# binli123/dsmil-wsi

Hardware: AMD Instinct MI355X
Metric: bags/sec aggregated (10kx512) (higher is better)
Workload: dtype f32; 1 GPU; DSMIL aggregator forward (FCLayer+BClassifier), c16 weights C=1, 64 bags x 10000 x 512 fp32 per GPU per pass, HBM-resident; bags_per_pass_per_gpu=64, rows=10000, feats=512, classes=1, tile_rows=128, parallelism=bag-sharded x1, streams=3, distinct_batches=3, logits_form=1, device_cus=256, persistent_grid=256

## Files before the change

dsmil-wsi_amd/csrc/agg_fwd.hip:

```cpp

#include <hip/hip_runtime.h>
#include <stdint.h>
#include <math.h>
#include <stdio.h>
#include <stdlib.h>
#include <string.h>
#include <atomic>
#include "dsmil_hip.h"
#include "prof.h"

#include "agg_common.h"
#include "agg_split.h"
#include "agg_hs.h"
#include "agg_f2.h"
#include "agg_f3.h"
#include "agg_res.h"
#include "lds_attr.h"

namespace {

template <int VEC, bool GIVEN, typename T = float>
__device__ __forceinline__ void logits_tile(
    const T* __restrict__ feats, const int64_t* __restrict__ offsets,
    const float* __restrict__ fc_w, const float* __restrict__ fc_b,
// ... 220 lines not shown
            a1 += b1;
            if (want_max) {
#pragma unroll
                for (int m = 1; m < 8; m <<= 1) xm = fmaxf(xm, __shfl_xor(xm, m, 64));
                if (j == 0 && rbase + rr < Nb) rowmax[off0 + r] = xm;
            }
            if (j == 0 && rbase + rr < Nb) {
                float* o = classes_out + (off0 + r) * (long long)C;
                o[c0] = a0;
                if (CP == 2 && c1 != c0) o[c1] = a1;
            }
            if (better(a0, r, bv0, bi0)) { bv0 = a0; bi0 = r; }
            if (CP == 2 && better(a1, r, bv1, bi1)) { bv1 = a1; bi1 = r; }
        }
#pragma unroll
        for (int m = 8; m < 64; m <<= 1) {
            const float ov0 = __shfl_xor(bv0, m, 64);
            const long long oi0 = __shfl_xor(bi0, m, 64);
            if (better(ov0, oi0, bv0, bi0)) { bv0 = ov0; bi0 = oi0; }
            if constexpr (CP == 2) {
                const float ov1 = __shfl_xor(bv1, m, 64);
                const long long oi1 = __shfl_xor(bi1, m, 64);
                if (better(ov1, oi1, bv1, bi1)) { bv1 = ov1; bi1 = oi1; }
            }
        }
        __syncthreads();
        if (lane == 0) { s_v[wave] = bv0; s_i[wave] = bi0; s_v[4 + wave] = bv1; s_i[4 + wave] = bi1; }
        __syncthreads();
        if (tid < 2 && (tid == 0 || c1 != c0)) {
            const int h = tid * 4;
            float bv = s_v[h];
            long long bi = s_i[h];
            for (int w = 1; w < 4; ++w)
                if (better(s_v[h + w], s_i[h + w], bv, bi)) { bv = s_v[h + w]; bi = s_i[h + w]; }
            const int c = tid ? c1 : c0;
            part_val[slot * C + c] = bv;
            part_idx[slot * C + c] = bi;
        }
    }
}

template <int CP>
__global__ __launch_bounds__(256, 6) void k_logits_pipe(
    const bf16_t* __restrict__ feats, const int64_t* __restrict__ offsets,
    const float* __restrict__ fc_w, const float* __restrict__ fc_b, float* __restrict__ classes_out,
    float* __restrict__ part_val, long long* __restrict__ part_idx, int bag0,
    int r0, const int* __restrict__ tile_pre, int n_bags) {
    constexpr int K = 512, SEG = 64;
    __shared__ __attribute__((aligned(16))) float s_w[CP * K];
    __shared__ float s_v[8];
    __shared__ int s_i[8];
    int bag = bag0 + (int)blockIdx.y, tile = (int)blockIdx.x;
    if (tile_pre) {
        if ((int)blockIdx.x >= tile_pre[n_bags]) return;
        const int b = tile_owner(tile_pre, n_bags, (int)blockIdx.x);
        bag = bag0 + b;
        tile = (int)blockIdx.x - tile_pre[b];
    }
    const long long off0 = offsets[bag];
    const long long Nbl = offsets[bag + 1] - off0;
    const long long row0l = (long long)tile * r0;
    if (row0l >= Nbl) return;
    const int Nb = (int)Nbl, row0 = (int)row0l;
    const int tid = threadIdx.x, lane = tid & 63, wave = tid >> 6;
    const int j = lane & 7, rr = lane >> 3;
    const int ngrp = r0 >> 5, rpw = r0 >> 2;
    const int wbase = row0 + wave * rpw;
    int ng = 0;
    if (wbase < Nb) { const int left = (Nb - wbase + 7) >> 3; ng = left < ngrp ? left : ngrp; }
    for (int i = tid; i < CP * K; i += 256) s_w[i] = fc_w[i];
    __syncthreads();
    const float b0 = fc_b[0], b1 = fc_b[CP - 1];
    float bv0 = -INFINITY, bv1 = -INFINITY;
    int bi0 = 0x7fffffff, bi1 = 0x7fffffff;
    if (ng > 0) {
        typedef StreamVec<bf16_t> SV;
        const bf16_t* fbase = feats + j * 8;
        auto row_of = [&](int g) { const int r = wbase + g * 8 + rr; return r < Nb ? r : Nb - 1; };
        auto ptr_of = [&](int r) { return fbase + (off0 + r) * (long long)K; };
        SV va[4], vb[4];
        float a0 = 0.f, a1 = 0.f;
        const unsigned wad = (unsigned)(size_t)(__attribute__((address_space(3))) float*)s_w + j * 32;
        auto piece = [&](const SV& v, auto off_tag) {
            constexpr int OFF = decltype(off_tag)::value;
            f32x4 wa, wb, wc, wd;
            if constexpr (CP == 2) {
                asm volatile("ds_read_b128 %0, %6 offset:%7\n\tds_read_b128 %1, %6 offset:%8\n\t"
                             "ds_read_b128 %2, %6 offset:%9\n\tds_read_b128 %3, %6 offset:%10\n\ts_waitcnt lgkmcnt(0)"
                             : "=&v"(wa), "=&v"(wb), "=&v"(wc), "=&v"(wd), "+v"(a0), "+v"(a1)
                             : "v"(wad), "n"(OFF), "n"(OFF + 16), "n"(OFF + K * 4), "n"(OFF + K * 4 + 16) : "memory");
            } else {
                asm volatile("ds_read_b128 %0, %3 offset:%4\n\tds_read_b128 %1, %3 offset:%5\n\ts_waitcnt lgkmcnt(0)"
                             : "=&v"(wa), "=&v"(wb), "+v"(a0) : "v"(wad), "n"(OFF), "n"(OFF + 16) : "memory");
            }
#pragma unroll
            for (int e = 0; e < 4; ++e) a0 = fmaf(v.at(e), wa[e], a0);
#pragma unroll
            for (int e = 0; e < 4; ++e) a0 = fmaf(v.at(4 + e), wb[e], a0);
            if constexpr (CP == 2) {
#pragma unroll
                for (int e = 0; e < 4; ++e) a1 = fmaf(v.at(e), wc[e], a1);
#pragma unroll
                for (int e = 0; e < 4; ++e) a1 = fmaf(v.at(4 + e), wd[e], a1);
            }
        };
        auto consume_lo = [&](const SV (&v)[4]) {
            piece(v[0], std::integral_constant<int, 0 * 256>{}); piece(v[1], std::integral_constant<int, 1 * 256>{});
            piece(v[2], std::integral_constant<int, 2 * 256>{}); piece(v[3], std::integral_constant<int, 3 * 256>{});
        };
        auto consume_hi = [&](const SV (&v)[4]) {
            piece(v[0], std::integral_constant<int, 4 * 256>{}); piece(v[1], std::integral_constant<int, 5 * 256>{});
            piece(v[2], std::integral_constant<int, 6 * 256>{}); piece(v[3], std::integral_constant<int, 7 * 256>{});
        };
        auto finish_rows = [&](int g, int r) {
#pragma unroll
            for (int m = 1; m < 8; m <<= 1) {
                a0 += __shfl_xor(a0, m, 64);
                if constexpr (CP == 2) a1 += __shfl_xor(a1, m, 64);
            }
            a0 += b0;
            a1 += b1;
            if (j == 0 && wbase + g * 8 + rr < Nb) {
                float* o = classes_out + (off0 + r) * (long long)CP;
                o[0] = a0;
                if constexpr (CP == 2) o[1] = a1;
            }
            if (a0 > bv0 || (a0 == bv0 && r < bi0)) { bv0 = a0; bi0 = r; }
            if (CP == 2 && (a1 > bv1 || (a1 == bv1 && r < bi1))) { bv1 = a1; bi1 = r; }
            a0 = 0.f;
            a1 = 0.f;
        };
        int r = row_of(0);
        const bf16_t* x = ptr_of(r);
#pragma unroll
        for (int u = 0; u < 4; ++u) va[u].load(x + u * SEG);
#pragma unroll 1
        for (int g = 0; g + 1 < ng; ++g) {
            const int rn = row_of(g + 1);
            const bf16_t* xn = ptr_of(rn);
#pragma unroll
            for (int u = 0; u < 4; ++u) vb[u].load(x + (4 + u) * SEG);
            consume_lo(va);
#pragma unroll
            for (int u = 0; u < 4; ++u) va[u].load(xn + u * SEG);
            consume_hi(vb);
            finish_rows(g, r);
            r = rn;
            x = xn;
        }
#pragma unroll
        for (int u = 0; u < 4; ++u) vb[u].load(x + (4 + u) * SEG);
        consume_lo(va);
        consume_hi(vb);
        finish_rows(ng - 1, r);
    }
#pragma unroll
    for (int m = 8; m < 64; m <<= 1) {
        const float ov0 = __shfl_xor(bv0, m, 64);
        const int oi0 = __shfl_xor(bi0, m, 64);
        if (ov0 > bv0 || (ov0 == bv0 && oi0 < bi0)) { bv0 = ov0; bi0 = oi0; }
        if constexpr (CP == 2) {
            const float ov1 = __shfl_xor(bv1, m, 64);
            const int oi1 = __shfl_xor(bi1, m, 64);
            if (ov1 > bv1 || (ov1 == bv1 && oi1 < bi1)) { bv1 = ov1; bi1 = oi1; }
        }
    }
    if (lane == 0) { s_v[wave] = bv0; s_i[wave] = bi0; s_v[4 + wave] = bv1; s_i[4 + wave] = bi1; }
    __syncthreads();
    if (tid < CP) {
        const int h = tid * 4;
        float bv = s_v[h];
        int bi = s_i[h];
        for (int w = 1; w < 4; ++w)
            if (s_v[h + w] > bv || (s_v[h + w] == bv && s_i[h + w] < bi)) { bv = s_v[h + w]; bi = s_i[h + w]; }
        const long long slot = off0 / r0 + bag + tile;
        part_val[slot * CP + tid] = bv;
        part_idx[slot * CP + tid] = bi == 0x7fffffff ? 0x7fffffffffffffffLL : (long long)bi;
    }
}

template <int VEC, typename T = float, bool PRE = false>
__device__ __forceinline__ void qmax_block(
    const T* __restrict__ feats, const int64_t* __restrict__ offsets,
    const float* __restrict__ part_val, const long long* __restrict__ part_idx,
    const float* __restrict__ q0_w, const float* __restrict__ q0_b,
    const float* __restrict__ q2_w, const float* __restrict__ q2_b,
    float* __restrict__ qmax, int64_t* __restrict__ idx_out, int K, int C, int nonlinear,
    int bag, int c, float* s_v, long long* s_i, float* s_h, int mode = 0, float* __restrict__ best_val_out = nullptr,
    const int64_t* __restrict__ rowmap = nullptr, int r0 = R0) {
    const long long off0 = mode == 2 ? 0 : offsets[bag];
    const long long Nb = mode == 2 ? C : offsets[bag + 1] - off0;
    const int lane = threadIdx.x & 63, wave = threadIdx.x >> 6;
    const int nwv = (int)blockDim.x >> 6;
    const int upw = QD / nwv;
    const long long slot0 = off0 / r0 + bag;
    const long long ntile = mode == 2 ? 0 : (Nb + r0 - 1) / r0;
    f32x4 w1r[PRE ? 32 : 1];
    float w2r[PRE ? 32 : 1];
    bool pre = false;
    float bv = -INFINITY;
    long long bi = 0x7fffffffffffffffLL;
    long long t_next = threadIdx.x;
    if constexpr (PRE) {
        pre = K == 512 && nwv == 8 && nonlinear && VEC == 4;
        if (pre) {
            if (t_next < ntile) {
                bv = part_val[(slot0 + t_next) * C + c];
                bi = part_idx[(slot0 + t_next) * C + c];
                t_next += blockDim.x;
            }
            __builtin_amdgcn_sched_barrier(0);
#pragma unroll
            for (int jb = 0; jb < 2; ++jb)
#pragma unroll
                for (int kk = 0; kk < 2; ++kk)
#pragma unroll
                    for (int u = 0; u < 8; ++u)
                        w1r[(jb * 2 + kk) * 8 + u] = *reinterpret_cast<const f32x4*>(q0_w + (long long)(wave * 16 + jb * 8 + u) * 512 + kk * 256 + lane * 4);
#pragma unroll
            for (int jb = 0; jb < 2; ++jb)
#pragma unroll
                for (int u = 0; u < 8; ++u) {
                    const float* wr = q2_w + (long long)(wave * 16 + jb * 8 + u) * QD;
                    w2r[(jb * 8 + u) * 2] = wr[lane];
                    w2r[(jb * 8 + u) * 2 + 1] = wr[lane + 64];
                }
            __builtin_amdgcn_sched_barrier(0);
        }
    }
    for (long long t = t_next; t < ntile; t += blockDim.x) {
        const float v = part_val[(slot0 + t) * C + c];
        const long long i = part_idx[(slot0 + t) * C + c];
        if (better(v, i, bv, bi)) { bv = v; bi = i; }
    }
#pragma unroll
    for (int o = 32; o >= 1; o >>= 1) {
        const float ov = __shfl_xor(bv, o, 64);
        const long long oi = __shfl_xor(bi, o, 64);
        if (better(ov, oi, bv, bi)) { bv = ov; bi = oi; }
    }
    if (lane == 0) { s_v[wave] = bv; s_i[wave] = bi; }
    __syncthreads();
    bv = s_v[0]; bi = s_i[0];
    for (int w = 1; w < nwv; ++w)
        if (better(s_v[w], s_i[w], bv, bi)) { bv = s_v[w]; bi = s_i[w]; }
    long long best = mode == 2 ? c : bi;
    if (best < 0 || best >= Nb) best = 0;
    if (threadIdx.x == 0 && mode != 2) {
        idx_out[(long long)bag * C + c] = best;
        if (best_val_out) best_val_out[(long long)bag * C + c] = bv;
    }
    if (mode == 1) return;
    const T* x = feats + (mode == 2 ? best : phys_row(rowmap, off0 + best)) * (long long)K;
    if (PRE && pre) {
        const f32x4 xv0 = load4<VEC, T>(x, lane * 4, K), xv1 = load4<VEC, T>(x, 256 + lane * 4, K);
#pragma unroll
        for (int jb = 0; jb < 2; ++jb) {
            float acc[8] = {0.f, 0.f, 0.f, 0.f, 0.f, 0.f, 0.f, 0.f};
#pragma unroll
            for (int kk = 0; kk < 2; ++kk) {
                const f32x4 xv = kk ? xv1 : xv0;
#pragma unroll
                for (int u = 0; u < 8; ++u) {
                    const f32x4 wv = w1r[(jb * 2 + kk) * 8 + u];
#pragma unroll
                    for (int e = 0; e < 4; ++e) acc[u] = fmaf(xv[e], wv[e], acc[u]);
                }
            }
#pragma unroll
            for (int u = 0; u < 8; ++u) {
                const float a = fmaxf(wave_sum(acc[u]) + q0_b[wave * 16 + jb * 8 + u], 0.f);
                if (lane == 0) s_h[wave * 16 + jb * 8 + u] = a;
            }
        }
        __syncthreads();
        float* out = qmax + ((long long)bag * C + c) * QD;
        const float h0 = s_h[lane], h1 = s_h[lane + 64];
#pragma unroll
        for (int jb = 0; jb < 2; ++jb) {
            float acc[8];
#pragma unroll
            for (int u = 0; u < 8; ++u) acc[u] = fmaf(h0, w2r[(jb * 8 + u) * 2], h1 * w2r[(jb * 8 + u) * 2 + 1]);
#pragma unroll
            for (int u = 0; u < 8; ++u) {
                const float a = wave_sum(acc[u]) + q2_b[wave * 16 + jb * 8 + u];
                if (lane == 0) out[wave * 16 + jb * 8 + u] = tanhf(a);
            }
        }
        return;
    }
    for (int jb = 0; jb < upw; jb += 8) {
        float acc[8] = {0.f, 0.f, 0.f, 0.f, 0.f, 0.f, 0.f, 0.f};
        const float* wr = q0_w + (long long)(wave * upw + jb) * K;
        for (int k0 = 0; k0 < K; k0 += 256) {
            const int k = k0 + lane * 4;
            const f32x4 xv = load4<VEC, T>(x, k, K);
#pragma unroll
            for (int u = 0; u < 8; ++u) {
                const f32x4 wv = load4<VEC>(wr + (long long)u * K, k, K);
#pragma unroll
                for (int e = 0; e < 4; ++e) acc[u] = fmaf(xv[e], wv[e], acc[u]);
            }
        }
#pragma unroll
        for (int u = 0; u < 8; ++u) {
            float a = wave_sum(acc[u]) + q0_b[wave * upw + jb + u];
// ... 931 lines not shown
}

int dsmil_fc_forward_rows(const float* feats, int64_t total_rows, int32_t K, int32_t C, const float* fc_w,
                          const float* fc_b, float* classes, const int64_t* rowmap, void* stream) {
    if (!feats || !fc_w || !fc_b || !classes || total_rows <= 0 || K <= 0 || C <= 0) return DSMIL_E_INVALID;
    hipStream_t st = (hipStream_t)stream;
    long long blocks = (total_rows + 3) / 4;
    if (blocks > 4096) blocks = 4096;
    const bool v4 = (K % 4 == 0) && (((uintptr_t)feats | (uintptr_t)fc_w) % 16 == 0);
    if (v4) hipLaunchKernelGGL(k_fc<4>, dim3((unsigned)blocks), dim3(256), 0, st, feats, fc_w, fc_b, classes, (long long)total_rows, K, C, rowmap);
    else hipLaunchKernelGGL(k_fc<1>, dim3((unsigned)blocks), dim3(256), 0, st, feats, fc_w, fc_b, classes, (long long)total_rows, K, C, rowmap);
    return hipGetLastError() == hipSuccess ? DSMIL_OK : DSMIL_E_LAUNCH;
}

void dsmil_agg_forward_leftovers(void* ws, int32_t n_bags, int64_t total_rows, int32_t K, int32_t Kv, int32_t C,
                                 const void** packed_split, const float** qmax, const float** pred_part, int* pred_blocks) {
    const WsLayout L = ws_layout(n_bags, total_rows, total_rows, K, Kv, C, pick_nw(n_bags, total_rows) * 32);
    if (pred_part) *pred_part = (const float*)((char*)ws + L.pred_part);
    if (pred_blocks) *pred_blocks = (int)L.nchunk_max;
    if (packed_split) *packed_split = (pick_nw(n_bags, total_rows) != 8 && mlp_mode()) ? (const void*)((char*)ws + L.wsplit) : nullptr;
    if (qmax) *qmax = (const float*)((char*)ws + L.qmax);
}

extern "C" {

int dsmil_abi_version(void) { return DSMIL_ABI_VERSION; }

int dsmil_agg_mlp_form(void) { return mlp_mode(); }
int dsmil_agg_batch_form(int mode) {
    if (mode >= 0 && mode <= 2) return g_use_f2.exchange(mode);
    return g_use_f2.load();
}
int dsmil_agg_logits_form(int mode) {
    if (mode >= 0 && mode <= 2) return g_logits_form.exchange(mode);
    return g_logits_form.load();
}
int dsmil_agg_persistent_grid(int n) {
    if (n >= 1 && n <= 1024) return g_persistent_grid.exchange(n);
    return g_persistent_grid.load();
}
int dsmil_device_cus(void) { return device_cus(); }
int dsmil_agg_inline_query(int mode) {
    if (mode == 0 || mode == 1) return g_inline_query.exchange(mode);
    return g_inline_query.load();
}

const char* dsmil_strerror(int code) {
    switch (code) {
        case DSMIL_OK: return "ok";
        case DSMIL_E_INVALID: return "invalid argument";
        case DSMIL_E_UNSUPPORTED: return "unsupported shape or dtype";
        case DSMIL_E_WORKSPACE: return "workspace too small";
        case DSMIL_E_LAUNCH: return "kernel launch failed";
        case DSMIL_E_ALIGN: return "pointer not aligned";
        default: return "unknown error";
    }
}

int dsmil_agg_tile_rows(int32_t n_bags, int64_t total_rows) { return pick_nw(n_bags, total_rows) * 32; }

size_t dsmil_agg_workspace_bytes(int32_t n_bags, int64_t total_rows, int32_t K, int32_t Kv,
                                 int32_t C) {
    (void)K;
    if (n_bags <= 0 || total_rows <= 0 || Kv <= 0 || C <= 0) return 0;
    return ws_layout(n_bags, total_rows, total_rows, K, Kv, C, pick_nw(n_bags, total_rows) * 32).total;
}

int dsmil_fc_forward(const float* feats, int64_t total_rows, int32_t K, int32_t C,
                     const float* fc_w, const float* fc_b, float* classes, void* stream) {
    return dsmil_fc_forward_rows(feats, total_rows, K, C, fc_w, fc_b, classes, nullptr, stream);
}

__global__ void k_set_offsets2(int64_t* off, long long N) { off[0] = 0; off[1] = N; }

static bool fwd_v4(const void* feats, const void* vals, const dsmil_agg_params* p) {
    return (p->K % 4 == 0) && (p->Kv % 4 == 0) &&
           (((uintptr_t)feats | (uintptr_t)vals | (uintptr_t)p->q0_w | (uintptr_t)p->fc_w |
             (uintptr_t)(p->nonlinear ? p->q2_w : p->q0_w)) % 16 == 0);
}

struct ShardCtl {
    int phase = 0;
    const float* crit_rows = nullptr;
    float* best_val = nullptr;
    float* ml_out = nullptr;
    bool skip_pred = false;
    const TrainPrologueJob* job = nullptr;
    const void* packed_f2 = nullptr;
};

static int agg_forward_impl(const void* feats, const void* vals, const int64_t* offsets,
                            int32_t n_bags, int64_t total_rows, int64_t max_rows, const dsmil_agg_params* p,
                            const void* packed_bf16, bool bf16, const float* classes_in, float* classes_out,
                            float* A, float* B, float* pred, int64_t* idx, void* ws, size_t ws_bytes,
                            void* stream, const ShardCtl& sh = ShardCtl(), const void* packed_split = nullptr,
                            const int64_t* rowmap = nullptr) {
    if (!feats || !p || !ws) return DSMIL_E_INVALID;
    if (sh.phase == 0 && (!offsets || !A || !B || (!pred && !sh.skip_pred) || !idx)) return DSMIL_E_INVALID;
    if (sh.phase == 1 && (!classes_out || !idx || !sh.best_val)) return DSMIL_E_INVALID;
    if (sh.phase == 2 && (!A || !B || !sh.crit_rows || !sh.ml_out)) return DSMIL_E_INVALID;
    if (n_bags <= 0 || total_rows <= 0 || max_rows <= 0 || max_rows > total_rows) return DSMIL_E_INVALID;
    if (p->K <= 0 || p->Kv <= 0 || p->C <= 0) return DSMIL_E_INVALID;
    if (!p->q0_w || !p->q0_b || !p->fcc_w || !p->fcc_b) return DSMIL_E_INVALID;
    if (p->nonlinear && (!p->q2_w || !p->q2_b)) return DSMIL_E_INVALID;
    if (sh.phase != 2 && !classes_in && (!p->fc_w || !p->fc_b || !classes_out)) return DSMIL_E_INVALID;
    if (bf16 && !packed_bf16) return DSMIL_E_INVALID;
    if (n_bags > 65535) return DSMIL_E_UNSUPPORTED;
    if (!vals) vals = feats;
    if (vals == feats && p->Kv != p->K) return DSMIL_E_INVALID;
    if (((uintptr_t)ws % 256) || ((uintptr_t)p->q0_b % 16) || (p->nonlinear && ((uintptr_t)p->q2_b % 16)))
        return DSMIL_E_ALIGN;
    const int K = p->K, Kv = p->Kv, C = p->C;
    if (bf16 && ((K % 8) || (Kv % 4) || ((uintptr_t)feats % 16) || ((uintptr_t)vals % 8) ||
                 ((uintptr_t)packed_bf16 % 16)))
        return DSMIL_E_UNSUPPORTED;
    const int NW = pick_nw(n_bags, total_rows);
    const int BM = NW * 32;
    const WsLayout L = ws_layout(n_bags, total_rows, max_rows, K, Kv, C, BM);
    if (ws_bytes < L.total) return DSMIL_E_WORKSPACE;
    hipStream_t st = (hipStream_t)stream;
    char* w8 = (char*)ws;
    if (sh.phase) {
        int64_t* off2 = (int64_t*)(w8 + L.off2);
        hipLaunchKernelGGL(k_set_offsets2, dim3(1), dim3(1), 0, st, off2, (long long)total_rows);
        if (hipGetLastError() != hipSuccess) return DSMIL_E_LAUNCH;
        offsets = off2;
    }
    float* part_val = (float*)(w8 + L.part_val);
    long long* part_idx = (long long*)(w8 + L.part_idx);
    float* qmax = (float*)(w8 + L.qmax);
    float* part_ml = (float*)(w8 + L.part_ml);
    float* part_B = (float*)(w8 + L.part_B);
    float* pred_part = (float*)(w8 + L.pred_part);
    const float* f32 = (const float*)feats;
    const bf16_t* b16 = (const bf16_t*)feats;

    const bool v4 = bf16 || fwd_v4(feats, vals, p);
    const bool w4 = (K % 4 == 0) && (((uintptr_t)p->q0_w | (uintptr_t)p->fc_w) % 16 == 0);
    AttendArgs a{feats, vals, (const bf16_t*)packed_bf16, offsets, p->q0_w, p->q0_b, p->q2_w, p->q2_b, qmax, A,
                 part_ml, part_B, K, Kv, C, p->nonlinear, 0, 0, rowmap};
#ifdef DSMIL_EXPERIMENTS
    static const int expt = expt_env("DSMIL_EXPT"), logits_old = expt_env("DSMIL_LOGITS_OLD"), no_hs = expt_env("DSMIL_NO_HS"),
                     no_qmi = expt_env("DSMIL_NO_QMI"), no_f2 = expt_env("DSMIL_NO_F2");
    a.expt = expt;
#else
    constexpr int logits_old = 0, no_hs = 0, no_qmi = 0, no_f2 = 0;
#endif
    int seg_per = 0, seg_T = 0;
    bool lean_tail = false;
    int hs_bm = 0;
    {
        const int b0 = 0, nb = n_bags;
        const bool stream_ok = !classes_in && !logits_old && ((bf16 && (K % 8 == 0)) || (!bf16 && v4));
        const bool lpipe = bf16 && stream_ok && !logits_old && K == 512 && C <= 2 && NW == 4 && sh.phase == 0 &&
                           !rowmap && max_rows < 0x7fffffffLL && coresident_wanted(st);
        const int r0 = lpipe ? PIPE_R0 : (NW == 1 && stream_ok && sh.phase != 2) ? 32 : R0;
        const int qmax_t = lpipe ? PIPE_QT : QMAX_T;
        lean_tail = lpipe;
        bool use_hs = !bf16 && NW == 1 && v4 && !no_hs && mlp_mode() == 6;
#ifdef DSMIL_EXPERIMENTS
        if (a.expt & 8) use_hs = false;
#endif
        const bool use_f2 = !bf16 && NW == 4 && v4 && !no_f2 && mlp_mode() == 6 && stream_ok && sh.phase == 0 && vals == feats &&
                            (K % 128 == 0) && K <= 16 * F2_MAXSTEPS && g_use_f2.load(std::memory_order_relaxed);
        float* rowmax = use_f2 ? (float*)(w8 + L.rowmax) : nullptr;
        const bool qm_inline = use_hs && stream_ok && sh.phase == 0 && !no_qmi && g_inline_query.load(std::memory_order_relaxed) &&
                               hs_inline_fits(max_rows, nb, C);
        int* qflag = qm_inline ? (int*)(w8 + L.qflag) : nullptr;
        dim3 grid((unsigned)((max_rows + r0 - 1) / r0), (unsigned)nb);
        int* tile_pre_a = nullptr;
        int* tile_pre_l = nullptr;
        if (NW == 4 && stream_ok && sh.phase == 0 && (long long)max_rows * nb != (long long)total_rows &&
            total_rows / 32 + nb < 0x7fffffffLL) {
            tile_pre_a = (int*)(w8 + L.tile_pre);
            tile_pre_l = tile_pre_a + (nb + 1);
            hipLaunchKernelGGL(k_tile_prefix, dim3(1), dim3(1024), 0, st, offsets, nb, bf16 ? RS_BM : F3_BM, r0, tile_pre_a, tile_pre_l);
            if (hipGetLastError() != hipSuccess) return DSMIL_E_LAUNCH;
        }
        const dim3 grid_l = tile_pre_l ? dim3((unsigned)(total_rows / r0 + nb), 1u) : grid;
        if (sh.phase == 2) {}
        else if (classes_in) hipLaunchKernelGGL((k_logits_argmax<1, true, float>), grid, dim3(256), 0, st, f32, offsets, p->fc_w, p->fc_b, classes_in, classes_out, part_val, part_idx, K, C, b0, rowmap);
        else if (bf16 && (K % 8 == 0) && !logits_old) {
            const size_t ldsw = (size_t)(C >= 2 ? 2 : 1) * (((K + 63) / 64 + 1) * 64) * sizeof(float);
            if (lpipe) {
                if (C == 2) hipLaunchKernelGGL(k_logits_pipe<2>, grid_l, dim3(256), 0, st, b16, offsets, p->fc_w, p->fc_b, classes_out, part_val, part_idx, b0, r0, tile_pre_l, nb);
                else hipLaunchKernelGGL(k_logits_pipe<1>, grid_l, dim3(256), 0, st, b16, offsets, p->fc_w, p->fc_b, classes_out, part_val, part_idx, b0, r0, tile_pre_l, nb);
            }
            else if (C >= 2) hipLaunchKernelGGL((k_logits_stream<2, bf16_t>), grid_l, dim3(256), ldsw, st, b16, offsets, p->fc_w, p->fc_b, classes_out, part_val, part_idx, K, C, b0, rowmap, r0, (int*)nullptr, TrainPrologueJob{}, (float*)nullptr, tile_pre_l, nb);
            else hipLaunchKernelGGL((k_logits_stream<1, bf16_t>), grid_l, dim3(256), ldsw, st, b16, offsets, p->fc_w, p->fc_b, classes_out, part_val, part_idx, K, C, b0, rowmap, r0, (int*)nullptr, TrainPrologueJob{}, (float*)nullptr, tile_pre_l, nb);
        }
        else if (bf16 && w4) hipLaunchKernelGGL((k_logits_argmax<4, false, bf16_t>), grid, dim3(256), 0, st, b16, offsets, p->fc_w, p->fc_b, classes_in, classes_out, part_val, part_idx, K, C, b0, rowmap);
        else if (bf16) hipLaunchKernelGGL((k_logits_argmax<1, false, bf16_t>), grid, dim3(256), 0, st, b16, offsets, p->fc_w, p->fc_b, classes_in, classes_out, part_val, part_idx, K, C, b0, rowmap);
        else if (v4 && !logits_old) {
            const size_t ldsw = (size_t)(C >= 2 ? 2 : 1) * (((K + 31) / 32 + 1) * 32) * sizeof(float);
            const TrainPrologueJob job = sh.job ? *sh.job : TrainPrologueJob{};
            dim3 gridj(grid_l.x + (unsigned)job.blocks, grid_l.y);
            if (C >= 2) hipLaunchKernelGGL((k_logits_stream<2, float>), gridj, dim3(256), ldsw, st, f32, offsets, p->fc_w, p->fc_b, classes_out, part_val, part_idx, K, C, b0, rowmap, r0, qflag, job, rowmax, tile_pre_l, nb);
            else hipLaunchKernelGGL((k_logits_stream<1, float>), gridj, dim3(256), ldsw, st, f32, offsets, p->fc_w, p->fc_b, classes_out, part_val, part_idx, K, C, b0, rowmap, r0, qflag, job, rowmax, tile_pre_l, nb);
        }
        else if (v4) hipLaunchKernelGGL((k_logits_argmax<4, false, float>), grid, dim3(256), 0, st, f32, offsets, p->fc_w, p->fc_b, classes_in, classes_out, part_val, part_idx, K, C, b0, rowmap);
        else hipLaunchKernelGGL((k_logits_argmax<1, false, float>), grid, dim3(256), 0, st, f32, offsets, p->fc_w, p->fc_b, classes_in, classes_out, part_val, part_idx, K, C, b0, rowmap);
        if (hipGetLastError() != hipSuccess) return DSMIL_E_LAUNCH;
        dim3 gq((unsigned)nb, (unsigned)C);
        if (sh.phase == 1) {
            if (v4) hipLaunchKernelGGL((k_qmax<4, float>), gq, dim3(QMAX_T), 0, st, f32, offsets, part_val, part_idx, p->q0_w, p->q0_b, p->q2_w, p->q2_b, qmax, idx, K, C, p->nonlinear, b0, 1, sh.best_val, rowmap, r0);
            else hipLaunchKernelGGL((k_qmax<1, float>), gq, dim3(QMAX_T), 0, st, f32, offsets, part_val, part_idx, p->q0_w, p->q0_b, p->q2_w, p->q2_b, qmax, idx, K, C, p->nonlinear, b0, 1, sh.best_val, rowmap, r0);
            return hipGetLastError() == hipSuccess ? DSMIL_OK : DSMIL_E_LAUNCH;
        }
        if (qm_inline) {
            a.qm_flag = qflag; a.qm_part_val = part_val; a.qm_part_idx = part_idx; a.qm_idx = idx; a.qm_r0 = r0;
        }
        else if (sh.phase == 2) {
            const bool r4 = (K % 4 == 0) && ((uintptr_t)sh.crit_rows % 16 == 0) && (((uintptr_t)p->q0_w) % 16 == 0);
            if (r4) hipLaunchKernelGGL((k_qmax<4, float>), gq, dim3(QMAX_T), 0, st, sh.crit_rows, offsets, part_val, part_idx, p->q0_w, p->q0_b, p->q2_w, p->q2_b, qmax, idx, K, C, p->nonlinear, b0, 2, (float*)nullptr);
            else hipLaunchKernelGGL((k_qmax<1, float>), gq, dim3(QMAX_T), 0, st, sh.crit_rows, offsets, part_val, part_idx, p->q0_w, p->q0_b, p->q2_w, p->q2_b, qmax, idx, K, C, p->nonlinear, b0, 2, (float*)nullptr);
        }
        else if (bf16 && w4) hipLaunchKernelGGL((k_qmax<4, bf16_t>), gq, dim3(qmax_t), 0, st, b16, offsets, part_val, part_idx, p->q0_w, p->q0_b, p->q2_w, p->q2_b, qmax, idx, K, C, p->nonlinear, b0, 0, (float*)nullptr, rowmap, r0);
        else if (bf16) hipLaunchKernelGGL((k_qmax<1, bf16_t>), gq, dim3(qmax_t), 0, st, b16, offsets, part_val, part_idx, p->q0_w, p->q0_b, p->q2_w, p->q2_b, qmax, idx, K, C, p->nonlinear, b0, 0, (float*)nullptr, rowmap, r0);
        else if (v4) hipLaunchKernelGGL((k_qmax<4, float>), gq, dim3(QMAX_T), 0, st, f32, offsets, part_val, part_idx, p->q0_w, p->q0_b, p->q2_w, p->q2_b, qmax, idx, K, C, p->nonlinear, b0, 0, (float*)nullptr, rowmap, r0);
        else hipLaunchKernelGGL((k_qmax<1, float>), gq, dim3(QMAX_T), 0, st, f32, offsets, part_val, part_idx, p->q0_w, p->q0_b, p->q2_w, p->q2_b, qmax, idx, K, C, p->nonlinear, b0, 0, (float*)nullptr, rowmap, r0);
        if (hipGetLastError() != hipSuccess) return DSMIL_E_LAUNCH;
        int rc;
        seg_per = seg_T = 0;
        const int mode = (NW == 8) ? 0 : mlp_mode();
        if (use_f2 && sh.packed_f2) {
            a.wpk = (const bf16_t*)sh.packed_f2;
        } else if (use_f2) {
            _Float16* wf2 = (_Float16*)(w8 + L.wf2);
            hipLaunchKernelGGL(k_pack_agg_f2, dim3(64), dim3(256), 0, st, p->q0_w, p->nonlinear ? p->q2_w : nullptr, wf2, K, 2 * ((K + 31) / 32));
            if (hipGetLastError() != hipSuccess) return DSMIL_E_LAUNCH;
            a.wpk = (const bf16_t*)wf2;
        } else if (!bf16 && mode && packed_split) {
            a.wpk = (const bf16_t*)packed_split;
        } else if (!bf16 && mode) {
            const int nks = 2 * ((K + 31) / 32);
            bf16_t* wsplit = (bf16_t*)(w8 + L.wsplit);
            hipLaunchKernelGGL(k_pack_agg_split, dim3(64), dim3(256), 0, st, p->q0_w, p->nonlinear ? p->q2_w : nullptr, wsplit, K, nks);
            if (hipGetLastError() != hipSuccess) return DSMIL_E_LAUNCH;
            a.wpk = wsplit;
        }
        bool bf16_dma = bf16 && NW == 4;
#ifdef DSMIL_EXPERIMENTS
        if (a.expt & 256) bf16_dma = false;
#endif
        bool bf16_res = bf16_dma && bf16_res_ok(a);
#ifdef DSMIL_EXPERIMENTS
        if (a.expt & 512) bf16_res = false;
#endif
        const bool use_f3 = use_f2 && p->nonlinear && C <= 2 && g_use_f2.load(std::memory_order_relaxed) == 2;
        if (tile_pre_a && (use_f3 || bf16_res)) {
            a.tile_pre = tile_pre_a;
            a.n_bags = nb;
        }
        if (use_f3) { rc = launch_attend_f3(a, rowmax, max_rows, total_rows, nb, st, &seg_per, &seg_T); hs_bm = F3_BM; }
        else if (use_f2) { rc = launch_attend_f2(a, rowmax, max_rows, nb, st); hs_bm = F2_BM; }
        else if (bf16_res) rc = launch_attend_bf16_res(a, max_rows, total_rows, nb, st, &seg_per, &seg_T);
        else if (bf16_dma) rc = launch_attend_bf16_dma(a, max_rows, nb, st);
        else if (bf16) rc = (NW == 4) ? launch_attend_bf16<4>(a, max_rows, nb, st) : launch_attend_bf16<1>(a, max_rows, nb, st);
#ifdef DSMIL_EXPERIMENTS
        else if (mode == 9 && NW == 4) rc = v4 ? launch_attend_split<4, 4, 9>(a, max_rows, nb, st) : launch_attend_split<4, 1, 9>(a, max_rows, nb, st);
        else if (mode == 9) rc = v4 ? launch_attend_split<1, 4, 9>(a, max_rows, nb, st) : launch_attend_split<1, 1, 9>(a, max_rows, nb, st);
        else if (mode == 6 && NW == 4 && v4 && (a.expt & 16)) rc = launch_attend_split<4, 4, 6, false, 16>(a, max_rows, nb, st);
        else if (mode == 6 && NW == 4 && v4 && (a.expt & 32)) rc = launch_attend_split<4, 4, 6, false, 32>(a, max_rows, nb, st);
        else if (mode == 6 && NW == 4 && v4 && (a.expt & 8)) rc = launch_attend_split<4, 4, 6, true>(a, max_rows, nb, st);
        else if (mode == 6 && NW == 1 && v4 && (a.expt & 8)) rc = launch_attend_split<1, 4, 6, true>(a, max_rows, nb, st);
#endif
        else if (mode == 6 && NW == 4) rc = v4 ? launch_attend_split<4, 4, 6>(a, max_rows, nb, st) : launch_attend_split<4, 1, 6>(a, max_rows, nb, st);
        else if (use_hs) { rc = launch_attend_hs(a, max_rows, nb, st); hs_bm = HS_BM; }
        else if (mode == 6) rc = v4 ? launch_attend_split<1, 4, 6>(a, max_rows, nb, st) : launch_attend_split<1, 1, 6>(a, max_rows, nb, st);
        else if (NW == 8) rc = launch_attend<8, 4>(a, max_rows, nb, st);
        else if (NW == 4) rc = v4 ? launch_attend<4, 4>(a, max_rows, nb, st) : launch_attend<4, 1>(a, max_rows, nb, st);
        else rc = v4 ? launch_attend<1, 4>(a, max_rows, nb, st) : launch_attend<1, 1>(a, max_rows, nb, st);
        if (rc != DSMIL_OK) return rc;
    }
    if (!DSMIL_EXPT_ON(a, 64)) {
        dim3 grid((unsigned)L.nchunk_max, (unsigned)n_bags);
        if (Kv % 4 == 0 && lean_tail && seg_per && !hs_bm)
            hipLaunchKernelGGL((k_finish<4, 2>), grid, dim3(256), 0, st, offsets, part_ml, part_B, p->fcc_w, A, B, pred_part, Kv, C, RS_BM, sh.ml_out, seg_per, seg_T, a.tile_pre);
        else if (Kv % 4 == 0)
            hipLaunchKernelGGL(k_finish<4>, grid, dim3(256), 0, st, offsets, part_ml, part_B, p->fcc_w, A, B, pred_part, Kv, C, hs_bm ? hs_bm : (seg_per ? RS_BM : BM), sh.ml_out, seg_per, seg_T, a.tile_pre);
        else
            hipLaunchKernelGGL(k_finish<1>, grid, dim3(256), 0, st, offsets, part_ml, part_B, p->fcc_w, A, B, pred_part, Kv, C, BM, sh.ml_out, 0, 0);
        if (hipGetLastError() != hipSuccess) return DSMIL_E_LAUNCH;
        if (sh.phase == 2 || sh.skip_pred) return DSMIL_OK;
        const int n = n_bags * C;
        hipLaunchKernelGGL(k_pred, dim3((unsigned)((n + 255) / 256)), dim3(256), 0, st, pred_part,
                           p->fcc_b, pred, C, (int)L.nchunk_max, n_bags);
        if (hipGetLastError() != hipSuccess) return DSMIL_E_LAUNCH;
    }
    return DSMIL_OK;
}

int dsmil_agg_forward(const float* feats, const float* vals, const int64_t* offsets,
                      int32_t n_bags, int64_t total_rows, int64_t max_rows,
                      const dsmil_agg_params* p, const float* classes_in, float* classes_out,
                      float* A, float* B, float* pred, int64_t* idx, void* ws, size_t ws_bytes,
                      void* stream) {
    return agg_forward_impl(feats, vals, offsets, n_bags, total_rows, max_rows, p, nullptr, false, classes_in,
                            classes_out, A, B, pred, idx, ws, ws_bytes, stream);
}

size_t dsmil_agg_packed_split_bytes(int32_t K, int32_t nonlinear) {
    if (K <= 0) return 0;
    return (size_t)(2 * ((K + 31) / 32) + (nonlinear ? 8 : 0)) * S3_CHUNK_F4 * 16;
}

int dsmil_agg_pack_split(const float* q0_w, const float* q2_w, int32_t K, void* packed, void* stream) {
    if (!q0_w || !packed || K <= 0) return DSMIL_E_INVALID;
    if ((uintptr_t)packed % 16) return DSMIL_E_ALIGN;
    hipLaunchKernelGGL(k_pack_agg_split, dim3(64), dim3(256), 0, (hipStream_t)stream, q0_w, q2_w, (bf16_t*)packed, K,
                       2 * ((K + 31) / 32));
    return hipGetLastError() == hipSuccess ? DSMIL_OK : DSMIL_E_LAUNCH;
}

size_t dsmil_agg_packed_f2_bytes(int32_t K) { return K <= 0 ? 0 : f2_image_bytes(K); }

int dsmil_agg_pack_f2(const float* q0_w, const float* q2_w, int32_t K, void* packed, void* stream) {
    if (!q0_w || !packed || K <= 0) return DSMIL_E_INVALID;
    if ((uintptr_t)packed % 16) return DSMIL_E_ALIGN;
    hipLaunchKernelGGL(k_pack_agg_f2, dim3(64), dim3(256), 0, (hipStream_t)stream, q0_w, q2_w, (_Float16*)packed, K,
                       2 * ((K + 31) / 32));
    return hipGetLastError() == hipSuccess ? DSMIL_OK : DSMIL_E_LAUNCH;
}

int dsmil_agg_forward_ex(const float* feats, const float* vals, const int64_t* offsets,
                         int32_t n_bags, int64_t total_rows, int64_t max_rows,
                         const dsmil_agg_params* p, const dsmil_agg_opts* opts, const float* classes_in,
                         float* classes_out, float* A, float* B, float* pred, int64_t* idx, void* ws,
                         size_t ws_bytes, void* stream) {
    const void* packed_split = opts ? opts->packed_split : nullptr;
    const int64_t* row_map = opts ? opts->row_map : nullptr;
    if (packed_split && ((uintptr_t)packed_split % 16)) return DSMIL_E_ALIGN;
    ShardCtl sh;
    sh.packed_f2 = opts ? opts->packed_f2 : nullptr;
    if (sh.packed_f2 && ((uintptr_t)sh.packed_f2 % 16)) return DSMIL_E_ALIGN;
    return agg_forward_impl(feats, vals, offsets, n_bags, total_rows, max_rows, p, nullptr, false, classes_in,
                            classes_out, A, B, pred, idx, ws, ws_bytes, stream, sh, packed_split, row_map);
}

}
bool dsmil_agg_forward_carries_prologue(const float* feats, int64_t total_rows, const dsmil_agg_params* p) {
#ifdef DSMIL_EXPERIMENTS
    static const int off = expt_env("DSMIL_LOGITS_OLD") | expt_env("DSMIL_NO_PROLOGUE_ROLE");
    if (off) return false;
#endif
    (void)total_rows;
    return feats && p && p->fc_w && fwd_v4(feats, feats, p);
}
int dsmil_agg_forward_nopred(const float* feats, const int64_t* offsets, int64_t total_rows, const dsmil_agg_params* p,
                             const dsmil_agg_opts* opts, float* classes_out, float* A, float* B, int64_t* idx, void* ws,
                             size_t ws_bytes, void* stream, const TrainPrologueJob* job) {
    ShardCtl sh;
    sh.skip_pred = true;
    if (job && !dsmil_agg_forward_carries_prologue(feats, total_rows, p)) return DSMIL_E_INVALID;
    sh.job = job;
    return agg_forward_impl(feats, nullptr, offsets, 1, total_rows, total_rows, p, nullptr, false, nullptr, classes_out, A, B,
                            nullptr, idx, ws, ws_bytes, stream, sh, opts ? opts->packed_split : nullptr,
                            opts ? opts->row_map : nullptr);
}
extern "C" {

static __global__ void k_loss_head(const float* __restrict__ classes, const float* __restrict__ pred,
                            const int64_t* __restrict__ idx, const float* __restrict__ label, int C,
                            float* __restrict__ loss, float* __restrict__ max_pred, float* __restrict__ g_pred,
                            float* __restrict__ g_max) {
    const int c = threadIdx.x;
    float l = 0.f;
    if (c < C) {
        const float y = label[c];
        const float zb = pred[c], zm = classes[idx[c] * (long long)C + c];
        const float lb = fmaxf(zb, 0.f) - zb * y + log1pf(expf(-fabsf(zb)));
        const float lm = fmaxf(zm, 0.f) - zm * y + log1pf(expf(-fabsf(zm)));
        l = 0.5f * (lb + lm) / (float)C;
        const float sb = 1.f / (1.f + expf(-zb)), sm = 1.f / (1.f + expf(-zm));
        if (max_pred) max_pred[c] = zm;
        if (g_pred) g_pred[c] = 0.5f * (sb - y) / (float)C;
        if (g_max) g_max[c] = 0.5f * (sm - y) / (float)C;
    }
    l = wave_sum(l);
    if (threadIdx.x == 0) *loss = l;
}

int dsmil_agg_loss_head(const float* classes, const float* pred, const int64_t* idx, const float* label,
                        int32_t C, float* loss, float* max_pred, float* g_pred, float* g_max, void* stream) {
    if (!classes || !pred || !idx || !label || !loss || C <= 0) return DSMIL_E_INVALID;
    if (C > 64) return DSMIL_E_UNSUPPORTED;
    hipLaunchKernelGGL(k_loss_head, dim3(1), dim3(64), 0, (hipStream_t)stream, classes, pred, idx, label, C, loss,
                       max_pred, g_pred, g_max);
    return hipGetLastError() == hipSuccess ? DSMIL_OK : DSMIL_E_LAUNCH;
}

int dsmil_agg_shard_argmax(const float* feats, int64_t rows, const dsmil_agg_params* p, float* classes_out,
                           float* best_val, int64_t* best_idx, void* ws, size_t ws_bytes, void* stream) {
    ShardCtl sh;
    sh.phase = 1;
    sh.best_val = best_val;
    return agg_forward_impl(feats, nullptr, nullptr, 1, rows, rows, p, nullptr, false, nullptr, classes_out, nullptr,
                            nullptr, nullptr, best_idx, ws, ws_bytes, stream, sh);
}

int dsmil_agg_shard_attend(const float* feats, const float* vals, int64_t rows, const dsmil_agg_params* p,
                           const float* crit_rows, float* A_unnorm, float* ml, float* B_unnorm, void* ws,
                           size_t ws_bytes, void* stream) {
    ShardCtl sh;
    sh.phase = 2;
    sh.crit_rows = crit_rows;
    sh.ml_out = ml;
    return agg_forward_impl(feats, vals, nullptr, 1, rows, rows, p, nullptr, false, nullptr, nullptr, A_unnorm,
                            B_unnorm, nullptr, nullptr, ws, ws_bytes, stream, sh);
}

size_t dsmil_agg_packed_bf16_bytes(int32_t K) {
    if (K <= 0) return 0;
    const size_t K64 = ((size_t)K + 63) / 64 * 64;
    return (QD * K64 + QD * QD) * sizeof(bf16_t) + (K64 / 64 + 2) * (size_t)BD_WCHUNK_F4 * 16;
}

int dsmil_agg_pack_bf16(const float* q0_w, const float* q2_w, int32_t K, void* packed, void* stream) {
    if (!q0_w || !packed || K <= 0) return DSMIL_E_INVALID;
    const int K64 = (K + 63) / 64 * 64;
    hipLaunchKernelGGL(k_pack_agg_bf16, dim3(512), dim3(256), 0, (hipStream_t)stream, q0_w, q2_w,
                       (bf16_t*)packed, K, K64);
    return hipGetLastError() == hipSuccess ? DSMIL_OK : DSMIL_E_LAUNCH;
}

int dsmil_agg_forward_bf16(const void* feats_bf16, const void* vals_bf16, const int64_t* offsets,
                           int32_t n_bags, int64_t total_rows, int64_t max_rows,
                           const dsmil_agg_params* p, const void* packed, const float* classes_in,
                           float* classes_out, float* A, float* B, float* pred, int64_t* idx, void* ws,
                           size_t ws_bytes, void* stream) {
    return agg_forward_impl(feats_bf16, vals_bf16, offsets, n_bags, total_rows, max_rows, p, packed, true,
// ... 5 lines not shown
```

Baseline: 108,100 bags/s.

## Add software-pipelined fp32 logits kernel and enable lean tail for f3 path

Adds an fp32 version of the pipelined logits kernel, specialised for K=512. It double-buffers row loads against FMAs that read weights from LDS, and also writes per-row abs-max for the f3 attend path. The new kernel is gated behind a logits_form==2 flag. When it is selected, the code uses the pipe tile size and qmax thread count and switches the finish kernel to the lean-tail variant with the f3 block size. The aim is to hide HBM latency in the logits pass. The trade-off is more inline-asm code paths and possible register pressure.

```diff
diff --git a/dsmil-wsi_amd/csrc/agg_fwd.hip b/dsmil-wsi_amd/csrc/agg_fwd.hip
--- a/dsmil-wsi_amd/csrc/agg_fwd.hip
+++ b/dsmil-wsi_amd/csrc/agg_fwd.hip
@@ -396,6 +396,154 @@
         for (int u = 0; u < 4; ++u) vb[u].load(x + (4 + u) * SEG);
         consume_lo(va);
         consume_hi(vb);
+        finish_rows(ng - 1, r);
+    }
+#pragma unroll
+    for (int m = 8; m < 64; m <<= 1) {
+        const float ov0 = __shfl_xor(bv0, m, 64);
+        const int oi0 = __shfl_xor(bi0, m, 64);
+        if (ov0 > bv0 || (ov0 == bv0 && oi0 < bi0)) { bv0 = ov0; bi0 = oi0; }
+        if constexpr (CP == 2) {
+            const float ov1 = __shfl_xor(bv1, m, 64);
+            const int oi1 = __shfl_xor(bi1, m, 64);
+            if (ov1 > bv1 || (ov1 == bv1 && oi1 < bi1)) { bv1 = ov1; bi1 = oi1; }
+        }
+    }
+    if (lane == 0) { s_v[wave] = bv0; s_i[wave] = bi0; s_v[4 + wave] = bv1; s_i[4 + wave] = bi1; }
+    __syncthreads();
+    if (tid < CP) {
+        const int h = tid * 4;
+        float bv = s_v[h];
+        int bi = s_i[h];
+        for (int w = 1; w < 4; ++w)
+            if (s_v[h + w] > bv || (s_v[h + w] == bv && s_i[h + w] < bi)) { bv = s_v[h + w]; bi = s_i[h + w]; }
+        const long long slot = off0 / r0 + bag + tile;
+        part_val[slot * CP + tid] = bv;
+        part_idx[slot * CP + tid] = bi == 0x7fffffff ? 0x7fffffffffffffffLL : (long long)bi;
+    }
+}
+
+template <int CP>
+__global__ __launch_bounds__(256, 6) void k_logits_pipe_f32(
+    const float* __restrict__ feats, const int64_t* __restrict__ offsets,
+    const float* __restrict__ fc_w, const float* __restrict__ fc_b, float* __restrict__ classes_out,
+    float* __restrict__ part_val, long long* __restrict__ part_idx, float* __restrict__ rowmax, int bag0,
+    int r0, const int* __restrict__ tile_pre, int n_bags) {
+    constexpr int K = 512, SEG = 32;
+    __shared__ __attribute__((aligned(16))) float s_w[CP * K];
+    __shared__ float s_v[8];
+    __shared__ int s_i[8];
+    int bag = bag0 + (int)blockIdx.y, tile = (int)blockIdx.x;
+    if (tile_pre) {
+        if ((int)blockIdx.x >= tile_pre[n_bags]) return;
+        const int b = tile_owner(tile_pre, n_bags, (int)blockIdx.x);
+        bag = bag0 + b;
+        tile = (int)blockIdx.x - tile_pre[b];
+    }
+    const long long off0 = offsets[bag];
+    const long long Nbl = offsets[bag + 1] - off0;
+    const long long row0l = (long long)tile * r0;
+    if (row0l >= Nbl) return;
+    const int Nb = (int)Nbl, row0 = (int)row0l;
+    const int tid = threadIdx.x, lane = tid & 63, wave = tid >> 6;
+    const int j = lane & 7, rr = lane >> 3;
+    const int ngrp = r0 >> 5, rpw = r0 >> 2;
+    const int wbase = row0 + wave * rpw;
+    int ng = 0;
+    if (wbase < Nb) { const int left = (Nb - wbase + 7) >> 3; ng = left < ngrp ? left : ngrp; }
+    for (int i = tid; i < CP * K; i += 256) s_w[i] = fc_w[i];
+    __syncthreads();
+    const float b0 = fc_b[0], b1 = fc_b[CP - 1];
+    float bv0 = -INFINITY, bv1 = -INFINITY;
+    int bi0 = 0x7fffffff, bi1 = 0x7fffffff;
+    if (ng > 0) {
+        typedef StreamVec<float> SV;
+        const float* fbase = feats + j * 4;
+        auto row_of = [&](int g) { const int r = wbase + g * 8 + rr; return r < Nb ? r : Nb - 1; };
+        auto ptr_of = [&](int r) { return fbase + (off0 + r) * (long long)K; };
+        SV va[4], vb[4];
+        float a0 = 0.f, a1 = 0.f, xm = 0.f;
+        const unsigned wad = (unsigned)(size_t)(__attribute__((address_space(3))) float*)s_w + j * 16;
+        auto piece = [&](const SV& v, auto off_tag) {
+            constexpr int OFF = decltype(off_tag)::value;
+            f32x4 wa, wc;
+            if constexpr (CP == 2) {
+                asm volatile("ds_read_b128 %0, %4 offset:%5\n\tds_read_b128 %1, %4 offset:%6\n\ts_waitcnt lgkmcnt(0)"
+                             : "=&v"(wa), "=&v"(wc), "+v"(a0), "+v"(a1) : "v"(wad), "n"(OFF), "n"(OFF + K * 4) : "memory");
+            } else {
+                asm volatile("ds_read_b128 %0, %2 offset:%3\n\ts_waitcnt lgkmcnt(0)"
+                             : "=&v"(wa), "+v"(a0) : "v"(wad), "n"(OFF) : "memory");
+            }
+#pragma unroll
+            for (int e = 0; e < 4; ++e) xm = fmaxf(xm, fabsf(v.at(e)));
+#pragma unroll
+            for (int e = 0; e < 4; ++e) a0 = fmaf(v.at(e), wa[e], a0);
+            if constexpr (CP == 2) {
+#pragma unroll
+                for (int e = 0; e < 4; ++e) a1 = fmaf(v.at(e), wc[e], a1);
+            }
+        };
+        auto consume = [&](const SV (&v)[4], auto q_tag) {
+            constexpr int Q = decltype(q_tag)::value;
+            piece(v[0], std::integral_constant<int, (4 * Q + 0) * 128>{}); piece(v[1], std::integral_constant<int, (4 * Q + 1) * 128>{});
+            piece(v[2], std::integral_constant<int, (4 * Q + 2) * 128>{}); piece(v[3], std::integral_constant<int, (4 * Q + 3) * 128>{});
+        };
+        auto load = [&](SV (&v)[4], const float* x, int q) {
+#pragma unroll
+            for (int u = 0; u < 4; ++u) v[u].load(x + (4 * q + u) * SEG);
+        };
+        using Q0 = std::integral_constant<int, 0>;
+        using Q1 = std::integral_constant<int, 1>;
+        using Q2 = std::integral_constant<int, 2>;
+        using Q3 = std::integral_constant<int, 3>;
+        auto finish_rows = [&](int g, int r) {
+#pragma unroll
+            for (int m = 1; m < 8; m <<= 1) {
+                a0 += __shfl_xor(a0, m, 64);
+                if constexpr (CP == 2) a1 += __shfl_xor(a1, m, 64);
+            }
+            a0 += b0;
+            a1 += b1;
+#pragma unroll
+            for (int m = 1; m < 8; m <<= 1) xm = fmaxf(xm, __shfl_xor(xm, m, 64));
+            if (j == 0 && wbase + g * 8 + rr < Nb) {
+                rowmax[off0 + r] = xm;
+                float* o = classes_out + (off0 + r) * (long long)CP;
+                o[0] = a0;
+                if constexpr (CP == 2) o[1] = a1;
+            }
+            if (a0 > bv0 || (a0 == bv0 && r < bi0)) { bv0 = a0; bi0 = r; }
+            if (CP == 2 && (a1 > bv1 || (a1 == bv1 && r < bi1))) { bv1 = a1; bi1 = r; }
+            a0 = 0.f;
+            a1 = 0.f;
+            xm = 0.f;
+        };
+        int r = row_of(0);
+        const float* x = ptr_of(r);
+        load(va, x, 0);
+#pragma unroll 1
+        for (int g = 0; g + 1 < ng; ++g) {
+            const int rn = row_of(g + 1);
+            const float* xn = ptr_of(rn);
+            load(vb, x, 1);
+            consume(va, Q0{});
+            load(va, x, 2);
+            consume(vb, Q1{});
+            load(vb, x, 3);
+            consume(va, Q2{});
+            load(va, xn, 0);
+            consume(vb, Q3{});
+            finish_rows(g, r);
+            r = rn;
+            x = xn;
+        }
+        load(vb, x, 1);
+        consume(va, Q0{});
+        load(va, x, 2);
+        consume(vb, Q1{});
+        load(vb, x, 3);
+        consume(va, Q2{});
+        consume(vb, Q3{});
         finish_rows(ng - 1, r);
     }
 #pragma unroll
@@ -1633,17 +1781,19 @@
     {
         const int b0 = 0, nb = n_bags;
         const bool stream_ok = !classes_in && !logits_old && ((bf16 && (K % 8 == 0)) || (!bf16 && v4));
-        const bool lpipe = bf16 && stream_ok && !logits_old && K == 512 && C <= 2 && NW == 4 && sh.phase == 0 &&
-                           !rowmap && max_rows < 0x7fffffffLL && coresident_wanted(st);
-        const int r0 = lpipe ? PIPE_R0 : (NW == 1 && stream_ok && sh.phase != 2) ? 32 : R0;
-        const int qmax_t = lpipe ? PIPE_QT : QMAX_T;
-        lean_tail = lpipe;
         bool use_hs = !bf16 && NW == 1 && v4 && !no_hs && mlp_mode() == 6;
 #ifdef DSMIL_EXPERIMENTS
         if (a.expt & 8) use_hs = false;
 #endif
         const bool use_f2 = !bf16 && NW == 4 && v4 && !no_f2 && mlp_mode() == 6 && stream_ok && sh.phase == 0 && vals == feats &&
                             (K % 128 == 0) && K <= 16 * F2_MAXSTEPS && g_use_f2.load(std::memory_order_relaxed);
+        const bool use_f3 = use_f2 && p->nonlinear && C <= 2 && g_use_f2.load(std::memory_order_relaxed) == 2;
+        const bool pipe_shape = stream_ok && !logits_old && K == 512 && C <= 2 && NW == 4 && sh.phase == 0 && !rowmap &&
+                                max_rows < 0x7fffffffLL && (bf16 || (use_f3 && !sh.job));
+        const bool lpipe = pipe_shape && (bf16 ? coresident_wanted(st) : g_logits_form.load(std::memory_order_relaxed) == 2);
+        const int r0 = lpipe ? PIPE_R0 : (NW == 1 && stream_ok && sh.phase != 2) ? 32 : R0;
+        const int qmax_t = lpipe ? PIPE_QT : QMAX_T;
+        lean_tail = lpipe;
         float* rowmax = use_f2 ? (float*)(w8 + L.rowmax) : nullptr;
         const bool qm_inline = use_hs && stream_ok && sh.phase == 0 && !no_qmi && g_inline_query.load(std::memory_order_relaxed) &&
                                hs_inline_fits(max_rows, nb, C);
@@ -1672,6 +1822,10 @@
         }
         else if (bf16 && w4) hipLaunchKernelGGL((k_logits_argmax<4, false, bf16_t>), grid, dim3(256), 0, st, b16, offsets, p->fc_w, p->fc_b, classes_in, classes_out, part_val, part_idx, K, C, b0, rowmap);
         else if (bf16) hipLaunchKernelGGL((k_logits_argmax<1, false, bf16_t>), grid, dim3(256), 0, st, b16, offsets, p->fc_w, p->fc_b, classes_in, classes_out, part_val, part_idx, K, C, b0, rowmap);
+        else if (lpipe) {
+            if (C == 2) hipLaunchKernelGGL(k_logits_pipe_f32<2>, grid_l, dim3(256), 0, st, f32, offsets, p->fc_w, p->fc_b, classes_out, part_val, part_idx, rowmax, b0, r0, tile_pre_l, nb);
+            else hipLaunchKernelGGL(k_logits_pipe_f32<1>, grid_l, dim3(256), 0, st, f32, offsets, p->fc_w, p->fc_b, classes_out, part_val, part_idx, rowmax, b0, r0, tile_pre_l, nb);
+        }
         else if (v4 && !logits_old) {
             const size_t ldsw = (size_t)(C >= 2 ? 2 : 1) * (((K + 31) / 32 + 1) * 32) * sizeof(float);
             const TrainPrologueJob job = sh.job ? *sh.job : TrainPrologueJob{};
@@ -1698,7 +1852,7 @@
         }
         else if (bf16 && w4) hipLaunchKernelGGL((k_qmax<4, bf16_t>), gq, dim3(qmax_t), 0, st, b16, offsets, part_val, part_idx, p->q0_w, p->q0_b, p->q2_w, p->q2_b, qmax, idx, K, C, p->nonlinear, b0, 0, (float*)nullptr, rowmap, r0);
         else if (bf16) hipLaunchKernelGGL((k_qmax<1, bf16_t>), gq, dim3(qmax_t), 0, st, b16, offsets, part_val, part_idx, p->q0_w, p->q0_b, p->q2_w, p->q2_b, qmax, idx, K, C, p->nonlinear, b0, 0, (float*)nullptr, rowmap, r0);
-        else if (v4) hipLaunchKernelGGL((k_qmax<4, float>), gq, dim3(QMAX_T), 0, st, f32, offsets, part_val, part_idx, p->q0_w, p->q0_b, p->q2_w, p->q2_b, qmax, idx, K, C, p->nonlinear, b0, 0, (float*)nullptr, rowmap, r0);
+        else if (v4) hipLaunchKernelGGL((k_qmax<4, float>), gq, dim3(qmax_t), 0, st, f32, offsets, part_val, part_idx, p->q0_w, p->q0_b, p->q2_w, p->q2_b, qmax, idx, K, C, p->nonlinear, b0, 0, (float*)nullptr, rowmap, r0);
         else hipLaunchKernelGGL((k_qmax<1, float>), gq, dim3(QMAX_T), 0, st, f32, offsets, part_val, part_idx, p->q0_w, p->q0_b, p->q2_w, p->q2_b, qmax, idx, K, C, p->nonlinear, b0, 0, (float*)nullptr, rowmap, r0);
         if (hipGetLastError() != hipSuccess) return DSMIL_E_LAUNCH;
         int rc;
@@ -1728,7 +1882,6 @@
 #ifdef DSMIL_EXPERIMENTS
         if (a.expt & 512) bf16_res = false;
 #endif
-        const bool use_f3 = use_f2 && p->nonlinear && C <= 2 && g_use_f2.load(std::memory_order_relaxed) == 2;
         if (tile_pre_a && (use_f3 || bf16_res)) {
             a.tile_pre = tile_pre_a;
             a.n_bags = nb;
@@ -1756,8 +1909,8 @@
     }
     if (!DSMIL_EXPT_ON(a, 64)) {
         dim3 grid((unsigned)L.nchunk_max, (unsigned)n_bags);
-        if (Kv % 4 == 0 && lean_tail && seg_per && !hs_bm)
-            hipLaunchKernelGGL((k_finish<4, 2>), grid, dim3(256), 0, st, offsets, part_ml, part_B, p->fcc_w, A, B, pred_part, Kv, C, RS_BM, sh.ml_out, seg_per, seg_T, a.tile_pre);
+        if (Kv % 4 == 0 && lean_tail && seg_per)
+            hipLaunchKernelGGL((k_finish<4, 2>), grid, dim3(256), 0, st, offsets, part_ml, part_B, p->fcc_w, A, B, pred_part, Kv, C, hs_bm ? hs_bm : RS_BM, sh.ml_out, seg_per, seg_T, a.tile_pre);
         else if (Kv % 4 == 0)
             hipLaunchKernelGGL(k_finish<4>, grid, dim3(256), 0, st, offsets, part_ml, part_B, p->fcc_w, A, B, pred_part, Kv, C, hs_bm ? hs_bm : (seg_per ? RS_BM : BM), sh.ml_out, seg_per, seg_T, a.tile_pre);
         else
```

After: 107,900 bags/s, median of 2. No clear change (-0.2%).
